# powturbo/Turbo-Range-Coder

Hardware: AMD Instinct MI355X
Metric: encode+decode MB/s, order-0 static-CDF rANS, 100 MB bytes (higher is better)
Workload: dtype u32; 1 GPU; text100m: 100000000 B/GPU, static-CDF rANS, 2 states (anscdf4senc/anscdf4sdec per chunk), tables in LDS, chunk 512 B, 1 lane = 1 chunk, 64 chunks/wave; codec=anscdf4s, chunk=512, bytes_per_gpu=100000000, compressed_bytes_per_gpu=64522350, steps_in_flight=1, exchange=none

## Files before the change

### turbo-range-coder_amd/csrc/trc_dir.hip

```cpp
#include <stdlib.h>
#include "trc_dev.h"
#include "trc_launch.h"

__global__ __launch_bounds__(256) void trc_static_prep_kernel(const u16 *__restrict__ cdf, u32 cdfnum,
                                                              u8 *__restrict__ tables)
{
    __shared__ u32 c[258];
    const u32 tid = threadIdx.x;
    for (u32 i = tid; i < 258; i += 256) c[i] = (i <= cdfnum) ? (u32)cdf[i] : TRC_PROB_ONE;
    __syncthreads();
    const u32 slot = blockIdx.x * 256 + tid;
    u32 x = 0, hi = 256;
    while (x + 1 < hi) { u32 mid = (x + hi) >> 1; if (c[mid] > slot) hi = mid; else x = mid; }
    tables[TRC_TAB_LUT + slot] = (u8)x;
    if (blockIdx.x == 0) {
        const u32 c0 = c[tid], f = c[tid + 1] - c0;
        uint4 e; u32 d;
        if (f == 0) {
            e = make_uint4(0u, 0u, 0xffffffffu, 0u); d = 1u << 16;
        } else if (f == 1) {
            e = make_uint4(0xffffffffu, TRC_PROB_ONE - 1u, 1u << 16, c0 + TRC_PROB_ONE - 1u); d = (1u << 16) | c0;
        } else {
            const u32 l = 32u - (u32)__clz((int)(f - 1));
            const u32 m = (u32)((((u64)1) << (31 + l)) / f) + 1u;
            e = make_uint4(m, (TRC_PROB_ONE - f) | ((l - 1u) << 24), f << 16, c0);
            d = (f << 16) | c0;
        }
        ((uint4 *)(tables + TRC_TAB_ENC))[tid] = e;
        ((u32 *)(tables + TRC_TAB_DEC))[tid] = d;
        for (u32 i = tid; i < 260; i += 256) ((u16 *)(tables + TRC_TAB_CDF))[i] = (u16)((i <= cdfnum) ? cdf[i] : TRC_PROB_ONE);
    }
}

void trc_launch_static_prep(const uint16_t *d_cdf, unsigned cdfnum, uint8_t *tables, hipStream_t s)
{
    hipLaunchKernelGGL(trc_static_prep_kernel, dim3(128), dim3(256), 0, s, d_cdf, (u32)cdfnum, tables);
}

__global__ __launch_bounds__(256) void trc_group_sums_kernel(const u32 *__restrict__ clen, u32 nchunks, u64 n, u32 chunk,
                                                             u32 *__restrict__ gsum)
{
    const u32 c = blockIdx.x * 256 + threadIdx.x;
    const u64 cstart = (u64)c * chunk;
    const u32 len = c < nchunks ? (u32)((n - cstart) < chunk ? (n - cstart) : chunk) : 0u;
    const u32 v = trc_wave_sum(c < nchunks ? trc_min(clen[c], len) : 0u);
    if (trc_lane() == 0 && (c >> 6) < ((nchunks + 63) >> 6)) gsum[c >> 6] = v;
}
void trc_launch_group_sums(const uint32_t *d_clen, uint32_t nchunks, size_t n, uint32_t chunk, uint32_t *gsum, hipStream_t s)
{
    hipLaunchKernelGGL(trc_group_sums_kernel, dim3((nchunks + 255) / 256), dim3(256), 0, s, d_clen, nchunks, (u64)n, chunk, gsum);
}

__global__ __launch_bounds__(1024) void trc_scan_groups_kernel(const u32 *__restrict__ gsum, u32 ngroups,
                                                               u64 *__restrict__ goff, u64 *__restrict__ total)
{
    __shared__ u32 wsum[16];
    __shared__ u64 base_s;
    const u32 tid = threadIdx.x, lane = tid & 63, wid = tid >> 6;
    if (tid == 0) base_s = 0;
    __syncthreads();
    for (u32 t0 = 0; t0 < ngroups; t0 += 1024) {
        const u32 i = t0 + tid;
        const u32 v = i < ngroups ? gsum[i] : 0u;
        const u32 inc = trc_wave_incl_scan(v);
        if (lane == 63) wsum[wid] = inc;
        __syncthreads();
        u32 wbase = 0;
        for (u32 k = 0; k < wid; k++) wbase += wsum[k];
        const u64 base = base_s;
        if (i < ngroups) goff[i] = base + wbase + inc - v;
        __syncthreads();
        if (tid == 1023) base_s = base + wbase + inc;
        __syncthreads();
    }
    if (tid == 0) { goff[ngroups] = base_s; if (total) *total = base_s; }
}
void trc_launch_scan_groups(const uint32_t *gsum, uint32_t ngroups, uint64_t *goff, uint64_t *d_total, hipStream_t s)
{
    TRC_LAUNCH_TIMED(trc_scan_groups_kernel, dim3(1), dim3(1024), 0, s, gsum, ngroups, goff, d_total);
}

__global__ __launch_bounds__(256) void trc_range_dir_kernel(const u32 *__restrict__ clen, u32 nchunks, u64 n, u32 chunk,
                                                            const u64 *__restrict__ goff_full, u32 first, u32 count,
                                                            u32 *__restrict__ gsum_sub, u64 *__restrict__ goff_sub)
{
    const u32 ngroups_sub = (count + 63u) >> 6, end = first + count;
    const u32 j = blockIdx.x * 4u + (threadIdx.x >> 6), lane = trc_lane();
    if (j > ngroups_sub) return;
    const u32 b = trc_min(first + 64u * j, end);
    auto clamped = [&](u32 c) -> u32 {
        const u64 left = n - (u64)c * chunk;
        return trc_min(clen[c], left < chunk ? (u32)left : chunk);
    };
    const u32 below = (b & ~63u) + lane, mine = b + lane;
    const u32 pre = trc_wave_sum(below < b ? clamped(below) : 0u);
    const u32 sum = trc_wave_sum(mine < end ? clamped(mine) : 0u);
    if (lane == 0) {
        goff_sub[j] = goff_full[b >> 6] + pre;
        if (j < ngroups_sub) gsum_sub[j] = sum;
    }
}
void trc_launch_range_dir(const uint32_t *d_clen, uint32_t nchunks, size_t n, uint32_t chunk, const uint64_t *goff_full,
                          uint32_t first, uint32_t count, uint32_t *gsum_sub, uint64_t *goff_sub, hipStream_t s)
{
    const uint32_t waves = (count + 63u) / 64u + 1u;
    hipLaunchKernelGGL(trc_range_dir_kernel, dim3((waves + 3u) / 4u), dim3(256), 0, s, d_clen, nchunks, (u64)n, chunk, goff_full,
                       first, count, gsum_sub, goff_sub);
}

#ifndef TRC_GATHER_VPT
#define TRC_GATHER_VPT 6
#endif
#ifndef TRC_GATHER_ATTR
#define TRC_GATHER_ATTR
#endif
#ifdef TRC_GATHER_PROF
__device__ unsigned long long trc_gat_wall[16 * 4096];
#endif
template <int PARTS>
__global__ __launch_bounds__(256) TRC_GATHER_ATTR void trc_gather_kernel(const u8 *__restrict__ in, u64 n, u32 chunk, u32 nchunks,
                                                         const u8 *__restrict__ scratch, u32 stride, int from_end,
                                                         const u8 *__restrict__ scratch2, u32 stride2, const u32 *__restrict__ aux,
                                                         const u32 *__restrict__ clen, const u64 *__restrict__ goff,
                                                         const u32 *__restrict__ gsum, u32 ngroups,
                                                         u8 *__restrict__ payload, u64 *__restrict__ total, u64 *__restrict__ goff_out)
{
    constexpr u32 NP = 64u * PARTS;
    constexpr u32 TPP = 256u / NP;
    constexpr u32 VPT = TRC_GATHER_VPT;
    __shared__ u32 ex_s[NP + 1];
    __shared__ u64 src_s[NP];
    __shared__ u64 base_s;
    const u32 g = blockIdx.x, tid = threadIdx.x, lane = tid & 63u, wid = tid >> 6;
#ifdef TRC_GATHER_PROF
    const u64 gw0 = wall_clock64();
#endif
    if (wid == 1 || blockDim.x == 64) {
        const u64 b = trc_group_base(goff, gsum, g);
        if (lane == 0) { base_s = b; if (goff_out) goff_out[g] = b; }
    }
    if (wid == 0) {
        const u32 c = g * 64 + lane;
        const u32 l = c < nchunks ? clen[c] : 0u;
        const u64 cstart = (u64)c * chunk;
        const u32 len = c < nchunks ? (u32)((n - cstart) < chunk ? (n - cstart) : chunk) : 0u;
        const bool raw = l == len;
        const u32 inc = trc_wave_incl_scan(l);
        if (PARTS == 1) {
            ex_s[lane] = inc - l;
            src_s[lane] = (u64)(uintptr_t)(raw ? in + cstart : from_end ? scratch + (u64)(c + 1) * stride - l : scratch + (u64)c * stride);
        } else {
            const u8 *a = scratch + (u64)c * stride;
            const u32 la = (raw || c >= nchunks) ? l : from_end >= 3 ? aux[2 * c] : 4u + *(const u32 *)a;
            ex_s[2 * lane] = inc - l; ex_s[2 * lane + 1] = inc - l + la;
            src_s[2 * lane] = (u64)(uintptr_t)(raw ? in + cstart : from_end == 4 ? scratch + (u64)(c + 1) * stride - la : a);
            src_s[2 * lane + 1] = (u64)(uintptr_t)(from_end == 3 ? scratch + (u64)(c + 1) * stride - (l - la) :
                                                   from_end == 4 ? scratch2 + (u64)(c + 1) * stride2 - (l - la) : scratch2 + (u64)c * stride2);
        }
        if (lane == 63) ex_s[NP] = inc;
    }
    __syncthreads();
#ifdef TRC_GATHER_PROF
    const u64 gw1 = wall_clock64();
#endif
    const u64 base = base_s;
    const u32 tot = ex_s[NP];
    if (total && g == ngroups - 1 && tid == 0) *total = base + tot;
    u8 *dst0 = payload + base;
    auto src_of = [&](u32 p) -> const u8 * { return (const u8 *)(uintptr_t)src_s[p]; };

    u32 head = (u32)((16u - ((uintptr_t)dst0 & 15u)) & 15u);
    if (head > tot) head = tot;
    const u32 nvec = (tot - head) >> 4;
    const u32 tail0 = head + (nvec << 4);
    const u32 sh = (u32)((64u - ((uintptr_t)dst0 & 63u)) & 63u);
    const u32 nsec = tot > sh ? (tot - sh) >> 6 : 0u;
    auto bytewise = [&](u32 dv, u32 kk) {
        const u8 *p = src_of(kk);
        for (u32 q = 0; q < 16; q++) {
            while (dv + q >= ex_s[kk + 1]) { kk++; p = src_of(kk); }
            dst0[dv + q] = p[dv + q - ex_s[kk]];
        }
    };
    auto piece_of = [&](u32 d) -> u32 {
        u32 lo = 0, hi = NP;
        while (lo + 1 < hi) { const u32 mid = (lo + hi) >> 1; if (ex_s[mid] <= d) lo = mid; else hi = mid; }
        return lo;
    };
    for (u32 b = tid; b < head + (tot - tail0); b += 256) {
        const u32 d = b < head ? b : tail0 + (b - head);
        const u32 lo = piece_of(d);
        dst0[d] = src_of(lo)[d - ex_s[lo]];
    }
    {
        const u32 nv1 = ((tot < sh ? tot : sh) - head) >> 4;
        const u32 nv2 = nvec - nv1 - 4u * nsec;
        const u32 e = tid - 64u;
        if (e < nv1 + nv2) {
            const u32 dv = e < nv1 ? head + (e << 4) : sh + (nsec << 6) + ((e - nv1) << 4);
            const u32 lo = piece_of(dv);
            if (dv + 16u <= ex_s[lo + 1]) *(uint4 *)(dst0 + dv) = trc_ld16_a2_global(src_of(lo) + (dv - ex_s[lo]));
            else bytewise(dv, lo);
        }
    }
    {
        const u32 k = tid / TPP, sub = tid % TPP;
        const u32 e0 = ex_s[k], e1 = ex_s[k + 1];
        const u32 s_lo = e0 <= sh ? 0u : (e0 - sh + 63u) >> 6;
        u32 s_hi = e1 <= sh ? 0u : (e1 - sh + 63u) >> 6;
        if (s_hi > nsec) s_hi = nsec;
        if (s_lo < s_hi) {
            const u8 *sa = src_of(k);
            const u8 *sb = k + 1 < NP ? src_of(k + 1) : sa;
            const u32 e2 = ex_s[k + 2 > NP ? NP : k + 2];
            const u32 pl = e1 - e0;
            const bool a16 = pl >= 16u;
            const bool b16 = k + 1 < NP && e2 - e1 >= 16u;
            constexpr u32 LV = 4u / TPP;
            enum { WHOLE, SPLICE, BYTES };
            uint4 la[LV], lb[LV];
            u32 ld[LV], lk[LV];
#pragma unroll
            for (int i = 0; i < (int)LV; i++) {
                const u32 d = sh + ((4u * (s_hi - 1u) + sub + TPP * (u32)i) << 4);
                ld[i] = d; lk[i] = BYTES;
                la[i] = make_uint4(0u, 0u, 0u, 0u); lb[i] = la[i];
                if (d + 16u <= e1) { la[i] = trc_ld16_a2_global(sa + (d - e0)); lk[i] = WHOLE; }
                else if (d < e1) { if (a16 && b16) { la[i] = trc_ld16_a2_global(sa + (pl - 16u)); lb[i] = trc_ld16_a2_global(sb); lk[i] = SPLICE; } }
                else if (d + 16u <= e2) { la[i] = trc_ld16_a2_global(sb + (d - e1)); lk[i] = WHOLE; }
            }
            const u32 u_hi = 4u * (s_hi - 1u);
            for (u32 u0 = 4u * s_lo + sub; u0 < u_hi; u0 += VPT * TPP) {
                uint4 a[VPT];
#pragma unroll
                for (int j = 0; j < (int)VPT; j++) {
                    const u32 u = u0 + TPP * (u32)j;
                    if (u < u_hi) a[j] = trc_ld16_a2_global(sa + (sh + (u << 4) - e0));
                }
#pragma unroll
                for (int j = 0; j < (int)VPT; j++) {
                    const u32 u = u0 + TPP * (u32)j;
                    if (u < u_hi) *(uint4 *)(dst0 + sh + (u << 4)) = a[j];
                }
            }
#pragma unroll
            for (int i = 0; i < (int)LV; i++) {
                if (lk[i] == WHOLE) *(uint4 *)(dst0 + ld[i]) = la[i];
                else if (lk[i] == SPLICE) *(uint4 *)(dst0 + ld[i]) = trc_splice16(la[i], lb[i], 16u - (e1 - ld[i]));
                else bytewise(ld[i], k);
            }
        }
    }
#ifdef TRC_GATHER_PROF
    {
        const u64 gw2 = wall_clock64();
        asm volatile("s_waitcnt vmcnt(0)" ::: "memory");
        const u64 gw3 = wall_clock64();
        if (lane == 0) { unsigned long long *w = trc_gat_wall + 16u * (g & 4095u) + 4u * (wid & 3u); w[0] = gw0; w[1] = gw1; w[2] = gw2; w[3] = gw3; }
    }
#endif
}
#ifdef TRC_GATHER_PROF
#include <stdio.h>
static void trc_gather_prof_report(u32 ngroups)
{
    static int calls = 0;
    if (++calls % 64 != 0) return;
    static unsigned long long wl[16 * 4096];
    (void)hipDeviceSynchronize();
    (void)hipMemcpyFromSymbol(wl, HIP_SYMBOL(trc_gat_wall), sizeof wl);
    const unsigned ng = ngroups < 4096u ? ngroups : 4096u;
    unsigned long long t0 = ~0ull;
    for (unsigned i = 0; i < 16 * ng; i += 4) if (wl[i] && wl[i] < t0) t0 = wl[i];
    double first_ready = 1e9, last_start = 0, sum_ready = 0, last_issue = 0, last_ack = 0, sum_ack = 0; unsigned cnt = 0;
    for (unsigned i = 0; i < 16 * ng; i += 4) {
        if (!wl[i]) continue;
        const double a = (wl[i] - t0) * 0.01, b = (wl[i + 1] - t0) * 0.01, c = (wl[i + 2] - t0) * 0.01, d = (wl[i + 3] - t0) * 0.01;
        if (a > last_start) last_start = a; if (b < first_ready) first_ready = b; if (c > last_issue) last_issue = c; if (d > last_ack) last_ack = d;
        sum_ready += b - a; sum_ack += d - a; cnt++;
    }
    fprintf(stderr, "[gather wall, us since the first wave's start] waves %u, last start %.2f; first table ready %.2f (mean %.2f after a wave's own start); last store issued %.2f, last store acknowledged %.2f (mean wave life %.2f)\n",
            cnt, last_start, first_ready, cnt ? sum_ready / cnt : 0.0, last_issue, last_ack, cnt ? sum_ack / cnt : 0.0);
}
#endif
void trc_launch_gather(const uint8_t *d_in, size_t n, uint32_t chunk, const TrcWork &w, TrcGather mode,
                       const uint32_t *d_clen, uint8_t *d_payload, uint64_t *d_total, hipStream_t s)
{
    const int from_end = mode;
    if (from_end >= 2)
        TRC_LAUNCH_TIMED((trc_gather_kernel<2>), dim3(w.ngroups), dim3(256), 0, s, d_in, (u64)n, chunk, w.nchunks,
                           w.scratch, w.stride, from_end >= 3 ? from_end : 0, w.scratch2, w.stride2, w.aux, d_clen, w.goff, w.gsum, w.ngroups,
                           d_payload, w.goff ? (u64 *)nullptr : d_total, w.goff ? (u64 *)nullptr : w.goff_area);
    else
        TRC_LAUNCH_TIMED((trc_gather_kernel<1>), dim3(w.ngroups), dim3(256), 0, s, d_in, (u64)n, chunk, w.nchunks,
                           w.scratch, w.stride, from_end, w.scratch2, w.stride2, w.aux, d_clen, w.goff, w.gsum, w.ngroups,
                           d_payload, w.goff ? (u64 *)nullptr : d_total, w.goff ? (u64 *)nullptr : w.goff_area);
#ifdef TRC_GATHER_PROF
    trc_gather_prof_report(w.ngroups);
#endif
}

#define TRC_HIST2_WAVE_LDS (128u * 16u * 4u)
#define TRC_HIST2_WAVES 16u
#define TRC_HIST2_ROUND_VECS 1023u
__global__ __launch_bounds__(1024) void trc_hist2_kernel(const u8 *__restrict__ in, u64 n, u64 *__restrict__ hist, u32 round_vecs)
{
    extern __shared__ __attribute__((aligned(16))) u8 smem[];
    typedef __attribute__((address_space(3))) u32 lds_u32;
    const u32 tid = threadIdx.x, lane = tid & 63u, wv = tid >> 6;
    u32 *mine = (u32 *)(smem + wv * TRC_HIST2_WAVE_LDS);
    u64 *tot = (u64 *)(smem + TRC_HIST2_WAVES * TRC_HIST2_WAVE_LDS);
    const u32 col = trc_lds_addr(mine) + (lane & 15u) * 4u;
    if (tid < 256u) tot[tid] = 0;
    const u64 nvec = n >> 4, stride = (u64)gridDim.x * 1024;
    const uint4 *v = (const uint4 *)in;
    auto count = [&](u32 w) __attribute__((always_inline)) {
#pragma unroll
        for (int k = 0; k < 4; k++) {
            const u32 a = (__builtin_amdgcn_ubfe(w, 8 * k + 1, 7) << 6) + col;
            const u32 inc = __umul24(__builtin_amdgcn_ubfe(w, 8 * k, 1), 0xffffu) + 1u;
            __hip_atomic_fetch_add((lds_u32 *)(uintptr_t)a, inc, __ATOMIC_RELAXED, __HIP_MEMORY_SCOPE_WAVEFRONT);
        }
    };
    auto count4 = [&](const uint4 q) __attribute__((always_inline)) { count(q.x); count(q.y); count(q.z); count(q.w); };
    for (u64 r0 = 0; r0 == 0 || r0 < nvec; r0 += stride * round_vecs) {
        for (u32 r = lane; r < 128u * 16u; r += 64u) mine[r] = 0;
        u64 i = r0 + (u64)blockIdx.x * 1024 + tid;
        u32 left = round_vecs;
        if (left >= 2u && i + stride < nvec) {
            uint4 q0 = v[i], q1 = v[i + stride];
            left -= 2u; i += 2 * stride;
            for (; left >= 2u && i + stride < nvec; left -= 2u, i += 2 * stride) {
                const uint4 n0 = v[i], n1 = v[i + stride];
                count4(q0); count4(q1);
                q0 = n0; q1 = n1;
            }
            count4(q0); count4(q1);
        }
        for (; left && i < nvec; left--, i += stride) count4(v[i]);
        if (r0 == 0 && blockIdx.x == 0 && wv == 0)
            for (u64 t = (nvec << 4) + lane; t < n; t += 64) {
                const u32 b = in[t];
                __hip_atomic_fetch_add((lds_u32 *)(uintptr_t)(col + (b >> 1) * 64u), (b & 1u) ? 0x10000u : 1u, __ATOMIC_RELAXED, __HIP_MEMORY_SCOPE_WAVEFRONT);
            }
        u32 lo0 = 0, hi0 = 0, lo1 = 0, hi1 = 0;
#pragma unroll
        for (u32 c4 = 0; c4 < 4u; c4++) {
            const uint4 a = *(const uint4 *)(mine + lane * 16u + c4 * 4u), b = *(const uint4 *)(mine + (lane + 64u) * 16u + c4 * 4u);
            lo0 += (a.x & 0xffffu) + (a.y & 0xffffu) + (a.z & 0xffffu) + (a.w & 0xffffu); hi0 += (a.x >> 16) + (a.y >> 16) + (a.z >> 16) + (a.w >> 16);
            lo1 += (b.x & 0xffffu) + (b.y & 0xffffu) + (b.z & 0xffffu) + (b.w & 0xffffu); hi1 += (b.x >> 16) + (b.y >> 16) + (b.z >> 16) + (b.w >> 16);
        }
        __syncthreads();
        atomicAdd((unsigned long long *)&tot[2 * lane], (unsigned long long)lo0);
        atomicAdd((unsigned long long *)&tot[2 * lane + 1], (unsigned long long)hi0);
        atomicAdd((unsigned long long *)&tot[2 * (lane + 64)], (unsigned long long)lo1);
        atomicAdd((unsigned long long *)&tot[2 * (lane + 64) + 1], (unsigned long long)hi1);
    }
    __syncthreads();
    if (tid < 256u) {
        const u32 bin = (tid + 37u * blockIdx.x) & 255u;
        if (tot[bin]) atomicAdd((unsigned long long *)&hist[bin], (unsigned long long)tot[bin]);
    }
}
__global__ __launch_bounds__(256) void trc_cdf_build_kernel(const u64 *__restrict__ hist, u64 n, u32 cdfnum,
                                                            u16 *__restrict__ cdf, int *__restrict__ status)
{
    __shared__ u64 f[256];
    __shared__ u32 pre[257];
    __shared__ int bad;
    const u32 tid = threadIdx.x;
    if (tid == 0) bad = 0;
    u64 v = 0;
    if (tid < cdfnum) { v = (hist[tid] << TRC_PROB_BITS) / n; if (!v) v = 1; }
    f[tid] = v;
    __syncthreads();
    if (tid == 0) {
        u64 best = 0, sum = 0; u32 bi = 0;
        for (u32 i = 0; i < cdfnum; i++) { sum += f[i]; if (f[i] > best) { best = f[i]; bi = i; } }
        f[bi] -= sum - TRC_PROB_ONE;
        u32 acc = 0; pre[0] = 0;
        for (u32 i = 0; i < cdfnum; i++) { acc = (acc + (u32)f[i]) & 0xffffu; pre[i + 1] = acc; }
    }
    __syncthreads();
    if (tid < cdfnum && pre[tid] >= pre[tid + 1]) atomicOr(&bad, 1);
    if (tid == 0 && pre[cdfnum] != (TRC_PROB_ONE & 0xffffu)) atomicOr(&bad, 1);
    __syncthreads();
    for (u32 i = tid; i <= cdfnum; i += 256) cdf[i] = (u16)pre[i];
    if (tid == 0) *status = bad ? -1 : (int)(n > 0x7fffffffull ? 0x7fffffffull : n);
}
void trc_launch_hist(const uint8_t *d_in, size_t n, uint64_t *d_hist, hipStream_t s)
{
    (void)hipMemsetAsync(d_hist, 0, 256 * sizeof(uint64_t), s);
    const size_t sm2 = TRC_HIST2_WAVES * TRC_HIST2_WAVE_LDS + 256u * sizeof(u64);
    u64 b2 = ((n >> 4) + 1023) / 1024;
    b2 = b2 < 1 ? 1 : b2 > 256 ? 256 : b2;
    TRC_RAISE_LDS_ONCE(trc_hist2_kernel, sm2);
    static const u32 rv = getenv("TRC_HIST_ROUND_VECS") ? (u32)atoi(getenv("TRC_HIST_ROUND_VECS")) : TRC_HIST2_ROUND_VECS;
    hipLaunchKernelGGL(trc_hist2_kernel, dim3((u32)b2), dim3(1024), sm2, s, d_in, (u64)n, d_hist,
                       rv >= 1u && rv <= TRC_HIST2_ROUND_VECS ? rv : TRC_HIST2_ROUND_VECS);
}
void trc_launch_cdf_build(const uint64_t *d_hist, size_t n_total, uint16_t *d_cdf, unsigned cdfnum, int32_t *d_status, hipStream_t s)
{
    hipLaunchKernelGGL(trc_cdf_build_kernel, dim3(1), dim3(256), 0, s, d_hist, (u64)n_total, (u32)cdfnum, d_cdf, d_status);
}
void trc_launch_cdfini(const uint8_t *d_in, size_t n, uint16_t *d_cdf, unsigned cdfnum,
                       int32_t *d_status, uint64_t *d_hist, hipStream_t s)
{
    trc_launch_hist(d_in, n, d_hist, s);
    trc_launch_cdf_build(d_hist, n, d_cdf, cdfnum, d_status, s);
}
```

Before: 736,900 MB/s.

## Make gather kernel persistent over groups with double-buffered piece tables

Each gather workgroup now handles several consecutive 64-chunk groups, sized from occupancy so the grid fits in one resident wave. The next group's clen/aux loads are issued before the current group's copy and stored into a second LDS buffer afterwards, and the running base offset is carried forward instead of recomputed per group. The aim is to cut per-block launch and prefix-lookup overhead and hide table-load latency. In exchange, blocks are serialised over groups, which can hurt load balance and adds a __syncthreads per group.

```diff
diff --git a/turbo-range-coder_amd/csrc/trc_dir.hip b/turbo-range-coder_amd/csrc/trc_dir.hip
--- a/turbo-range-coder_amd/csrc/trc_dir.hip
+++ b/turbo-range-coder_amd/csrc/trc_dir.hip
@@ -1,4 +1,5 @@
 #include <stdlib.h>
+#include <atomic>
 #include "trc_dev.h"
 #include "trc_launch.h"
 
@@ -122,133 +123,162 @@
                                                          const u8 *__restrict__ scratch, u32 stride, int from_end,
                                                          const u8 *__restrict__ scratch2, u32 stride2, const u32 *__restrict__ aux,
                                                          const u32 *__restrict__ clen, const u64 *__restrict__ goff,
-                                                         const u32 *__restrict__ gsum, u32 ngroups,
+                                                         const u32 *__restrict__ gsum, u32 ngroups, u32 gpw,
                                                          u8 *__restrict__ payload, u64 *__restrict__ total, u64 *__restrict__ goff_out)
 {
     constexpr u32 NP = 64u * PARTS;
     constexpr u32 TPP = 256u / NP;
     constexpr u32 VPT = TRC_GATHER_VPT;
-    __shared__ u32 ex_s[NP + 1];
-    __shared__ u64 src_s[NP];
+    __shared__ u32 ex_buf[2][NP + 1];
+    __shared__ u64 src_buf[2][NP];
     __shared__ u64 base_s;
-    const u32 g = blockIdx.x, tid = threadIdx.x, lane = tid & 63u, wid = tid >> 6;
+    const u32 tid0 = threadIdx.x, lane = tid0 & 63u, wid = tid0 >> 6;
+    const u32 g_first = blockIdx.x * gpw, g_end = trc_min(ngroups, g_first + gpw);
 #ifdef TRC_GATHER_PROF
     const u64 gw0 = wall_clock64();
 #endif
-    if (wid == 1 || blockDim.x == 64) {
-        const u64 b = trc_group_base(goff, gsum, g);
-        if (lane == 0) { base_s = b; if (goff_out) goff_out[g] = b; }
-    }
-    if (wid == 0) {
+    struct TabIn { u32 l, la; };
+    auto tab_load = [&](u32 g, u32 lane) -> TabIn {
         const u32 c = g * 64 + lane;
-        const u32 l = c < nchunks ? clen[c] : 0u;
+        TabIn t = { 0u, 0u };
+        if (c < nchunks) {
+            t.l = clen[c];
+            if (PARTS == 2) t.la = from_end >= 3 ? aux[2 * c] : 4u + *(const u32 *)(scratch + (u64)c * stride);
+        }
+        return t;
+    };
+    auto tab_store = [&](u32 g, u32 lane, const TabIn t, u32 *ex, u64 *src) {
+        const u32 c = g * 64 + lane;
+        const u32 l = t.l;
         const u64 cstart = (u64)c * chunk;
         const u32 len = c < nchunks ? (u32)((n - cstart) < chunk ? (n - cstart) : chunk) : 0u;
         const bool raw = l == len;
         const u32 inc = trc_wave_incl_scan(l);
         if (PARTS == 1) {
-            ex_s[lane] = inc - l;
-            src_s[lane] = (u64)(uintptr_t)(raw ? in + cstart : from_end ? scratch + (u64)(c + 1) * stride - l : scratch + (u64)c * stride);
+            ex[lane] = inc - l;
+            src[lane] = (u64)(uintptr_t)(raw ? in + cstart : from_end ? scratch + (u64)(c + 1) * stride - l : scratch + (u64)c * stride);
         } else {
             const u8 *a = scratch + (u64)c * stride;
-            const u32 la = (raw || c >= nchunks) ? l : from_end >= 3 ? aux[2 * c] : 4u + *(const u32 *)a;
-            ex_s[2 * lane] = inc - l; ex_s[2 * lane + 1] = inc - l + la;
-            src_s[2 * lane] = (u64)(uintptr_t)(raw ? in + cstart : from_end == 4 ? scratch + (u64)(c + 1) * stride - la : a);
-            src_s[2 * lane + 1] = (u64)(uintptr_t)(from_end == 3 ? scratch + (u64)(c + 1) * stride - (l - la) :
-                                                   from_end == 4 ? scratch2 + (u64)(c + 1) * stride2 - (l - la) : scratch2 + (u64)c * stride2);
-        }
-        if (lane == 63) ex_s[NP] = inc;
-    }
+            const u32 la = (raw || c >= nchunks) ? l : t.la;
+            ex[2 * lane] = inc - l; ex[2 * lane + 1] = inc - l + la;
+            src[2 * lane] = (u64)(uintptr_t)(raw ? in + cstart : from_end == 4 ? scratch + (u64)(c + 1) * stride - la : a);
+            src[2 * lane + 1] = (u64)(uintptr_t)(from_end == 3 ? scratch + (u64)(c + 1) * stride - (l - la) :
+                                                 from_end == 4 ? scratch2 + (u64)(c + 1) * stride2 - (l - la) : scratch2 + (u64)c * stride2);
+        }
+        if (lane == 63) ex[NP] = inc;
+    };
+    if (wid == 1 || blockDim.x == 64) {
+        const u64 b = trc_group_base(goff, gsum, g_first);
+        if (lane == 0) base_s = b;
+    }
+    if (wid == 0) tab_store(g_first, lane, tab_load(g_first, lane), ex_buf[0], src_buf[0]);
     __syncthreads();
 #ifdef TRC_GATHER_PROF
     const u64 gw1 = wall_clock64();
 #endif
-    const u64 base = base_s;
-    const u32 tot = ex_s[NP];
-    if (total && g == ngroups - 1 && tid == 0) *total = base + tot;
-    u8 *dst0 = payload + base;
-    auto src_of = [&](u32 p) -> const u8 * { return (const u8 *)(uintptr_t)src_s[p]; };
-
-    u32 head = (u32)((16u - ((uintptr_t)dst0 & 15u)) & 15u);
-    if (head > tot) head = tot;
-    const u32 nvec = (tot - head) >> 4;
-    const u32 tail0 = head + (nvec << 4);
-    const u32 sh = (u32)((64u - ((uintptr_t)dst0 & 63u)) & 63u);
-    const u32 nsec = tot > sh ? (tot - sh) >> 6 : 0u;
-    auto bytewise = [&](u32 dv, u32 kk) {
-        const u8 *p = src_of(kk);
-        for (u32 q = 0; q < 16; q++) {
-            while (dv + q >= ex_s[kk + 1]) { kk++; p = src_of(kk); }
-            dst0[dv + q] = p[dv + q - ex_s[kk]];
-        }
-    };
-    auto piece_of = [&](u32 d) -> u32 {
-        u32 lo = 0, hi = NP;
-        while (lo + 1 < hi) { const u32 mid = (lo + hi) >> 1; if (ex_s[mid] <= d) lo = mid; else hi = mid; }
-        return lo;
-    };
-    for (u32 b = tid; b < head + (tot - tail0); b += 256) {
-        const u32 d = b < head ? b : tail0 + (b - head);
-        const u32 lo = piece_of(d);
-        dst0[d] = src_of(lo)[d - ex_s[lo]];
-    }
-    {
-        const u32 nv1 = ((tot < sh ? tot : sh) - head) >> 4;
-        const u32 nv2 = nvec - nv1 - 4u * nsec;
-        const u32 e = tid - 64u;
-        if (e < nv1 + nv2) {
-            const u32 dv = e < nv1 ? head + (e << 4) : sh + (nsec << 6) + ((e - nv1) << 4);
-            const u32 lo = piece_of(dv);
-            if (dv + 16u <= ex_s[lo + 1]) *(uint4 *)(dst0 + dv) = trc_ld16_a2_global(src_of(lo) + (dv - ex_s[lo]));
-            else bytewise(dv, lo);
-        }
-    }
-    {
-        const u32 k = tid / TPP, sub = tid % TPP;
-        const u32 e0 = ex_s[k], e1 = ex_s[k + 1];
-        const u32 s_lo = e0 <= sh ? 0u : (e0 - sh + 63u) >> 6;
-        u32 s_hi = e1 <= sh ? 0u : (e1 - sh + 63u) >> 6;
-        if (s_hi > nsec) s_hi = nsec;
-        if (s_lo < s_hi) {
-            const u8 *sa = src_of(k);
-            const u8 *sb = k + 1 < NP ? src_of(k + 1) : sa;
-            const u32 e2 = ex_s[k + 2 > NP ? NP : k + 2];
-            const u32 pl = e1 - e0;
-            const bool a16 = pl >= 16u;
-            const bool b16 = k + 1 < NP && e2 - e1 >= 16u;
-            constexpr u32 LV = 4u / TPP;
-            enum { WHOLE, SPLICE, BYTES };
-            uint4 la[LV], lb[LV];
-            u32 ld[LV], lk[LV];
-#pragma unroll
-            for (int i = 0; i < (int)LV; i++) {
-                const u32 d = sh + ((4u * (s_hi - 1u) + sub + TPP * (u32)i) << 4);
-                ld[i] = d; lk[i] = BYTES;
-                la[i] = make_uint4(0u, 0u, 0u, 0u); lb[i] = la[i];
-                if (d + 16u <= e1) { la[i] = trc_ld16_a2_global(sa + (d - e0)); lk[i] = WHOLE; }
-                else if (d < e1) { if (a16 && b16) { la[i] = trc_ld16_a2_global(sa + (pl - 16u)); lb[i] = trc_ld16_a2_global(sb); lk[i] = SPLICE; } }
-                else if (d + 16u <= e2) { la[i] = trc_ld16_a2_global(sb + (d - e1)); lk[i] = WHOLE; }
+    u64 base = base_s;
+    for (u32 g = g_first; g < g_end; g++) {
+        const u32 *ex_s = ex_buf[(g - g_first) & 1u];
+        const u64 *src_s = src_buf[(g - g_first) & 1u];
+        const bool more = g + 1u < g_end;
+        u32 tid = tid0; asm volatile("" : "+v"(tid));
+        const u32 lane = tid & 63u, wid = tid >> 6;
+        TabIn nxt = { 0u, 0u };
+        if (more && wid == 0) nxt = tab_load(g + 1u, lane);
+        const u32 tot = ex_s[NP];
+        if (tid == 0) {
+            if (goff_out) goff_out[g] = base;
+            if (total && g == ngroups - 1) *total = base + tot;
+        }
+        u8 *dst0 = payload + base;
+        auto src_of = [&](u32 p) -> const u8 * { return (const u8 *)(uintptr_t)src_s[p]; };
+
+        u32 head = (u32)((16u - ((uintptr_t)dst0 & 15u)) & 15u);
+        if (head > tot) head = tot;
+        const u32 nvec = (tot - head) >> 4;
+        const u32 tail0 = head + (nvec << 4);
+        const u32 sh = (u32)((64u - ((uintptr_t)dst0 & 63u)) & 63u);
+        const u32 nsec = tot > sh ? (tot - sh) >> 6 : 0u;
+        auto bytewise = [&](u32 dv, u32 kk) {
+            const u8 *p = src_of(kk);
+            for (u32 q = 0; q < 16; q++) {
+                while (dv + q >= ex_s[kk + 1]) { kk++; p = src_of(kk); }
+                dst0[dv + q] = p[dv + q - ex_s[kk]];
             }
-            const u32 u_hi = 4u * (s_hi - 1u);
-            for (u32 u0 = 4u * s_lo + sub; u0 < u_hi; u0 += VPT * TPP) {
-                uint4 a[VPT];
-#pragma unroll
-                for (int j = 0; j < (int)VPT; j++) {
-                    const u32 u = u0 + TPP * (u32)j;
-                    if (u < u_hi) a[j] = trc_ld16_a2_global(sa + (sh + (u << 4) - e0));
+        };
+        auto piece_of = [&](u32 d) -> u32 {
+            u32 lo = 0, hi = NP;
+            while (lo + 1 < hi) { const u32 mid = (lo + hi) >> 1; if (ex_s[mid] <= d) lo = mid; else hi = mid; }
+            return lo;
+        };
+        for (u32 b = tid; b < head + (tot - tail0); b += 256) {
+            const u32 d = b < head ? b : tail0 + (b - head);
+            const u32 lo = piece_of(d);
+            dst0[d] = src_of(lo)[d - ex_s[lo]];
+        }
+        {
+            const u32 nv1 = ((tot < sh ? tot : sh) - head) >> 4;
+            const u32 nv2 = nvec - nv1 - 4u * nsec;
+            const u32 e = tid - 64u;
+            if (e < nv1 + nv2) {
+                const u32 dv = e < nv1 ? head + (e << 4) : sh + (nsec << 6) + ((e - nv1) << 4);
+                const u32 lo = piece_of(dv);
+                if (dv + 16u <= ex_s[lo + 1]) *(uint4 *)(dst0 + dv) = trc_ld16_a2_global(src_of(lo) + (dv - ex_s[lo]));
+                else bytewise(dv, lo);
+            }
+        }
+        {
+            const u32 k = tid / TPP, sub = tid % TPP;
+            const u32 e0 = ex_s[k], e1 = ex_s[k + 1];
+            const u32 s_lo = e0 <= sh ? 0u : (e0 - sh + 63u) >> 6;
+            u32 s_hi = e1 <= sh ? 0u : (e1 - sh + 63u) >> 6;
+            if (s_hi > nsec) s_hi = nsec;
+            if (s_lo < s_hi) {
+                const u8 *sa = src_of(k);
+                const u8 *sb = k + 1 < NP ? src_of(k + 1) : sa;
+                const u32 e2 = ex_s[k + 2 > NP ? NP : k + 2];
+                const u32 pl = e1 - e0;
+                const bool a16 = pl >= 16u;
+                const bool b16 = k + 1 < NP && e2 - e1 >= 16u;
+                constexpr u32 LV = 4u / TPP;
+                enum { WHOLE, SPLICE, BYTES };
+                uint4 la[LV], lb[LV];
+                u32 ld[LV], lk[LV];
+#pragma unroll
+                for (int i = 0; i < (int)LV; i++) {
+                    const u32 d = sh + ((4u * (s_hi - 1u) + sub + TPP * (u32)i) << 4);
+                    ld[i] = d; lk[i] = BYTES;
+                    la[i] = make_uint4(0u, 0u, 0u, 0u); lb[i] = la[i];
+                    if (d + 16u <= e1) { la[i] = trc_ld16_a2_global(sa + (d - e0)); lk[i] = WHOLE; }
+                    else if (d < e1) { if (a16 && b16) { la[i] = trc_ld16_a2_global(sa + (pl - 16u)); lb[i] = trc_ld16_a2_global(sb); lk[i] = SPLICE; } }
+                    else if (d + 16u <= e2) { la[i] = trc_ld16_a2_global(sb + (d - e1)); lk[i] = WHOLE; }
                 }
-#pragma unroll
-                for (int j = 0; j < (int)VPT; j++) {
-                    const u32 u = u0 + TPP * (u32)j;
-                    if (u < u_hi) *(uint4 *)(dst0 + sh + (u << 4)) = a[j];
+                const u32 u_hi = 4u * (s_hi - 1u);
+                for (u32 u0 = 4u * s_lo + sub; u0 < u_hi; u0 += VPT * TPP) {
+                    uint4 a[VPT];
+#pragma unroll
+                    for (int j = 0; j < (int)VPT; j++) {
+                        const u32 u = u0 + TPP * (u32)j;
+                        if (u < u_hi) a[j] = trc_ld16_a2_global(sa + (sh + (u << 4) - e0));
+                    }
+#pragma unroll
+                    for (int j = 0; j < (int)VPT; j++) {
+                        const u32 u = u0 + TPP * (u32)j;
+                        if (u < u_hi) *(uint4 *)(dst0 + sh + (u << 4)) = a[j];
+                    }
+                }
+#pragma unroll
+                for (int i = 0; i < (int)LV; i++) {
+                    if (lk[i] == WHOLE) *(uint4 *)(dst0 + ld[i]) = la[i];
+                    else if (lk[i] == SPLICE) *(uint4 *)(dst0 + ld[i]) = trc_splice16(la[i], lb[i], 16u - (e1 - ld[i]));
+                    else bytewise(ld[i], k);
                 }
             }
-#pragma unroll
-            for (int i = 0; i < (int)LV; i++) {
-                if (lk[i] == WHOLE) *(uint4 *)(dst0 + ld[i]) = la[i];
-                else if (lk[i] == SPLICE) *(uint4 *)(dst0 + ld[i]) = trc_splice16(la[i], lb[i], 16u - (e1 - ld[i]));
-                else bytewise(ld[i], k);
-            }
+        }
+        if (more) {
+            if (wid == 0) tab_store(g + 1u, lane, nxt, ex_buf[(g + 1u - g_first) & 1u], src_buf[(g + 1u - g_first) & 1u]);
+            __syncthreads();
+            base += tot;
         }
     }
 #ifdef TRC_GATHER_PROF
@@ -256,7 +286,7 @@
         const u64 gw2 = wall_clock64();
         asm volatile("s_waitcnt vmcnt(0)" ::: "memory");
         const u64 gw3 = wall_clock64();
-        if (lane == 0) { unsigned long long *w = trc_gat_wall + 16u * (g & 4095u) + 4u * (wid & 3u); w[0] = gw0; w[1] = gw1; w[2] = gw2; w[3] = gw3; }
+        if (lane == 0) { unsigned long long *w = trc_gat_wall + 16u * (blockIdx.x & 4095u) + 4u * (wid & 3u); w[0] = gw0; w[1] = gw1; w[2] = gw2; w[3] = gw3; }
     }
 #endif
 }
@@ -283,20 +313,40 @@
             cnt, last_start, first_ready, cnt ? sum_ready / cnt : 0.0, last_issue, last_ack, cnt ? sum_ack / cnt : 0.0);
 }
 #endif
+static u32 trc_gather_gpw(bool two, u32 ngroups)
+{
+    static const int env = getenv("TRC_GATHER_GPW") ? atoi(getenv("TRC_GATHER_GPW")) : 0;
+    if (env > 0) return (u32)env;
+    static std::atomic<u32> cap_s[2][64];
+    int dev = 0;
+    if (hipGetDevice(&dev) != hipSuccess || dev < 0 || dev > 63) return 1u;
+    u32 cap = cap_s[two][dev].load(std::memory_order_relaxed);
+    if (cap == 0u) {
+        int per_cu = 0, cus = 0;
+        const void *k = two ? (const void *)trc_gather_kernel<2> : (const void *)trc_gather_kernel<1>;
+        const bool ok = hipOccupancyMaxActiveBlocksPerMultiprocessor(&per_cu, k, 256, 0) == hipSuccess &&
+                        hipDeviceGetAttribute(&cus, hipDeviceAttributeMultiprocessorCount, dev) == hipSuccess && per_cu > 0 && cus > 0;
+        cap = ok ? (u32)per_cu * (u32)cus : ~0u;
+        cap_s[two][dev].store(cap, std::memory_order_relaxed);
+    }
+    return cap == ~0u || ngroups <= cap ? 1u : (ngroups + cap - 1u) / cap;
+}
 void trc_launch_gather(const uint8_t *d_in, size_t n, uint32_t chunk, const TrcWork &w, TrcGather mode,
                        const uint32_t *d_clen, uint8_t *d_payload, uint64_t *d_total, hipStream_t s)
 {
     const int from_end = mode;
-    if (from_end >= 2)
-        TRC_LAUNCH_TIMED((trc_gather_kernel<2>), dim3(w.ngroups), dim3(256), 0, s, d_in, (u64)n, chunk, w.nchunks,
-                           w.scratch, w.stride, from_end >= 3 ? from_end : 0, w.scratch2, w.stride2, w.aux, d_clen, w.goff, w.gsum, w.ngroups,
+    const bool two = from_end >= 2;
+    const u32 gpw = trc_gather_gpw(two, w.ngroups), grid = (w.ngroups + gpw - 1u) / gpw;
+    if (two)
+        TRC_LAUNCH_TIMED((trc_gather_kernel<2>), dim3(grid), dim3(256), 0, s, d_in, (u64)n, chunk, w.nchunks,
+                           w.scratch, w.stride, from_end >= 3 ? from_end : 0, w.scratch2, w.stride2, w.aux, d_clen, w.goff, w.gsum, w.ngroups, gpw,
                            d_payload, w.goff ? (u64 *)nullptr : d_total, w.goff ? (u64 *)nullptr : w.goff_area);
     else
-        TRC_LAUNCH_TIMED((trc_gather_kernel<1>), dim3(w.ngroups), dim3(256), 0, s, d_in, (u64)n, chunk, w.nchunks,
-                           w.scratch, w.stride, from_end, w.scratch2, w.stride2, w.aux, d_clen, w.goff, w.gsum, w.ngroups,
+        TRC_LAUNCH_TIMED((trc_gather_kernel<1>), dim3(grid), dim3(256), 0, s, d_in, (u64)n, chunk, w.nchunks,
+                           w.scratch, w.stride, from_end, w.scratch2, w.stride2, w.aux, d_clen, w.goff, w.gsum, w.ngroups, gpw,
                            d_payload, w.goff ? (u64 *)nullptr : d_total, w.goff ? (u64 *)nullptr : w.goff_area);
 #ifdef TRC_GATHER_PROF
-    trc_gather_prof_report(w.ngroups);
+    trc_gather_prof_report(grid);
 #endif
 }
 
```

Result: no change. 738,800 MB/s (median of 6 runs) (+0.3%).
